# LinXueyuanStdio/LaTeX_OCR

Measured on NVIDIA H100. Metric: formula-images/sec (train step, 128x512 px, seq<=150), higher is better.
Workload: dtype bf16

## Files before the change

### include/latex_ocr_b200.h

```cpp
#ifndef LATEX_OCR_B200_H
#define LATEX_OCR_B200_H

#include <stdint.h>

#ifdef __cplusplus
extern "C" {
#endif

#define LO_F32 0
#define LO_BF16 1

#define LO_OK 0
#define LO_EINVAL (-1)
#define LO_ECUDA (-2)
#define LO_ENOTSUP (-3)

#define LO_IMPL_SIMT 0
#define LO_IMPL_TC 1

int lo_version(void);
const char* lo_last_error(void);
int64_t lo_launch_count(void);
int lo_set_option(const char* name, int value);
int lo_get_option(const char* name);
// ... 38 lines not shown
               int N, int H, int W, int Cin, int Cout, int pad, int relu, int impl, void* stream);
int lo_conv3x3_wgrad(const void* x, const void* dy, float* dw, float* db, int dt,
                     int N, int H, int W, int Cin, int Cout, int pad, int impl, void* stream);
int lo_conv_weight_flip(const void* w, void* wt, int dt, int Cin, int Cout, void* stream);
int lo_maxpool_forward(const void* x, void* y, int dt, int N, int H, int W, int C, int kh, int kw, void* stream);
int lo_maxpool_backward(const void* x, const void* y, const void* dy, void* dx, int dt,
                        int N, int H, int W, int C, int kh, int kw, void* stream);
int lo_add_table(const void* y, const float* table, void* out, int dt, int N, int64_t HWC, void* stream);
int lo_relu_mask_cast(const float* g, const void* y, void* out, int dt, int64_t n, void* stream);

int64_t lo_attention_workspace_bytes(int B, int C);
int64_t lo_decoder_workspace_bytes(int B, int C);
int lo_attention_forward(const void* att1, const void* enc, int dt, const float* att2, int64_t att2_stride,
                         const float* wf, float* alpha, int64_t alpha_stride, float* ctx,
                         float* gate_pre, int64_t gate_stride, float* gctx,
                         int B, int R, int A, int C, void* work, void* stream);
int lo_attention_forward_mask(const void* att1, const void* enc, int dt, const float* att2, int64_t att2_stride,
                              const float* wf, float* alpha, int64_t alpha_stride, float* ctx,
                              float* gate_pre, int64_t gate_stride, float* gctx, uint8_t* relu_mask_out,
                              int B, int R, int A, int C, void* work, void* stream);

int lo_attention_backward(const void* att1, const void* enc, int dt, const float* att2, const float* gate, int64_t o1_stride,
                          const float* wf, const float* alpha, int64_t alpha_stride, const float* ctx, const float* dgctx,
                          int64_t dg_stride, const float* dreg, int64_t dreg_stride, const float* sreg, int64_t sreg_stride,
                          float* de, float* datt2, float* dgp, int64_t dcat_stride, float* dctx_out, float* dwf_part,
                          const uint8_t* relu_mask, int B, int R, int A, int C, void* work, void* stream);

int64_t lo_attention_step_workspace_bytes(int B, int R, int A, int C, int dt);
int lo_attention_step_backward(const void* enc, const void* att1, int dt, const float* h, const float* att2, const void* w_enc,
                               const void* w_dec, const float* wf, const float* alpha, const float* ctx, const float* dctx,
                               const float* dalpha, float* denc, float* dh, float* g_w_enc, float* g_b_enc, float* g_w_dec,
                               float* g_b_dec, float* g_w_full, float* g_b_full, float* de, float* datt2, void* datt1,
                               int B, int R, int A, int C, int D, int impl, void* work, void* stream);

typedef struct lo_decoder_args {
  int32_t B, T, R, C, A, D, E, V;
  int32_t dt;
  int32_t impl;
  int32_t has_dropout;
  int32_t ldl;
  float alpha_c;
  int32_t rows_per_img;
  int32_t phase;
  const int32_t* bt_host;
  const int64_t* caps;
  int64_t caps_stride;
  int64_t* fed;
  const float* ss_prob;
  const float* ss_u;
  const float* ss_temp;
  const float* ss_gu;
  const void* enc;
  const void* w_enc_att; const float* b_enc_att;
  const void* wcat1; const float* bcat1;
  const float* w_full;
  const void* emb;
  const void* w_ih; const float* b_ih;
  const void* w_init; const float* b_init;
  const void* w_fc; const float* b_fc;
  void* wbwd1;
  void* wbwd2;
  void* att1;
  float* ptab;
  float* mean;
  float* hall;
  float* call;
// ... 175 lines not shown
```

### latex_ocr_b200/csrc/lo_decoder.cu

```cuda
#include "lo_common.cuh"
#include "lo_ptx.cuh"

namespace lo {

#define LO_ATT_THREADS 256
#define LO_ATT_WARPS 8
#define LO_ATT_MAXSPLIT 16

static inline int att_splits(int B) {
  int s = (444 + B - 1) / B;
  if (s < 1) s = 1;
  if (s > LO_ATT_MAXSPLIT) s = LO_ATT_MAXSPLIT;
  return s;
}

__device__ __forceinline__ float ldcg_f(const float* p) { return __ldcg(p); }

template <typename T, int NV>
__global__ void __launch_bounds__(LO_ATT_THREADS) attention_fwd_kernel(
    const T* __restrict__ att1, const T* __restrict__ enc, const float* __restrict__ att2, int64_t att2_stride,
    const float* __restrict__ wf, float* __restrict__ alpha, int64_t alpha_stride, float* __restrict__ ctx,
    float* __restrict__ gate_pre, int64_t gate_stride, float* __restrict__ gctx, bf16* __restrict__ gctx_bf, int R, int nsplit,
    int* __restrict__ counters, float* __restrict__ partials, int rpi) {
  constexpr int CH = NV * 256;
// ... 207 lines not shown
  __shared__ float s_acc[LO_ATT_WARPS][CH];
  __shared__ int s_last;
#pragma unroll
  for (int j = 0; j < NV; j++)
#pragma unroll
    for (int i = 0; i < 8; i++) s_acc[wid][(j * 32 + lane) * 8 + i] = macc[j * 8 + i];
  __syncthreads();
  float* part = partials + ((int64_t)b * nsplit + sp) * (CH + 2);
  for (int c = threadIdx.x; c < CH; c += LO_ATT_THREADS) {
    float t = 0.f;
#pragma unroll
    for (int w = 0; w < LO_ATT_WARPS; w++) t += s_acc[w][c];
    part[2 + c] = t;
  }
  __threadfence();
  __syncthreads();
  if (threadIdx.x == 0) {
    const int ticket = atomicAdd(counters + b, 1);
    s_last = (ticket == nsplit - 1);
    if (s_last) counters[b] = 0;
  }
  __syncthreads();
  if (!s_last) return;
  __threadfence();
  const float* pb = partials + (int64_t)b * nsplit * (CH + 2);
  for (int c = threadIdx.x; c < CH; c += LO_ATT_THREADS) {
    float t = 0.f;
    for (int sidx = 0; sidx < nsplit; sidx++) t += ldcg_f(pb + (int64_t)sidx * (CH + 2) + 2 + c);
    datt2[(int64_t)b * dcat_stride + c] = t * wf[c];
    if (datt2_bf) datt2_bf[(int64_t)b * dcat_stride + c] = __float2bfloat16_rn(t * wf[c]);
  }
}

template <typename T, int WACC, int ACT = 0>
__global__ void __launch_bounds__(128) datt1_kernel(const T* __restrict__ att1, const float* __restrict__ out1,
                                                     int64_t o1_row, int64_t o1_step, const float* __restrict__ de,
                                                     const float* __restrict__ wf, T* __restrict__ datt1,
                                                     float* __restrict__ dwf, int Tn, int R, int A, int nchunk, int dwf_rows) {
  constexpr int TT = 32;
  __shared__ __align__(16) float s_a2[TT][64];
  __shared__ __align__(16) float s_de[TT][32];
  __shared__ float s_w[8][64];
  const int b = blockIdx.z, a0 = blockIdx.x * 64;
  const int tx = threadIdx.x % 16, ty = threadIdx.x / 16;
  float wacc[4] = {0.f, 0.f, 0.f, 0.f};
  for (int ch = 0; ch < nchunk; ch++) {
  const int r0 = (blockIdx.y * nchunk + ch) * 32;
  if (r0 >= R) break;
  float x[4][4], nx[4][4], acc[4][4];
#pragma unroll
  for (int i = 0; i < 4; i++) {
    const int r = r0 + ty * 4 + i;
#pragma unroll
    for (int j = 0; j < 4; j++) {
      acc[i][j] = 0.f;
      x[i][j] = (r < R) ? ldf(att1 + ((int64_t)b * R + r) * A + a0 + tx * 4 + j) : -INFINITY;
      nx[i][j] = -x[i][j];
    }
  }
  for (int t0 = 0; t0 < Tn; t0 += TT) {
    for (int i = threadIdx.x; i < TT * 64; i += 128) {
      const int tt = i / 64, a = i % 64;
      s_a2[tt][a] = (t0 + tt < Tn) ? out1[(int64_t)(t0 + tt) * o1_step + (int64_t)b * o1_row + a0 + a] : 0.f;
    }
    for (int i = threadIdx.x; i < TT * 32; i += 128) {
      const int tt = i / 32, r = i % 32;
      s_de[tt][r] = (t0 + tt < Tn && r0 + r < R) ? de[((int64_t)b * Tn + t0 + tt) * R + r0 + r] : 0.f;
    }
    __syncthreads();
#pragma unroll 4
    for (int tt = 0; tt < TT; tt++) {
      const float4 q = *reinterpret_cast<const float4*>(&s_a2[tt][tx * 4]);
      const float4 d4 = *reinterpret_cast<const float4*>(&s_de[tt][ty * 4]);
      const float a2v[4] = {q.x, q.y, q.z, q.w}, dv[4] = {d4.x, d4.y, d4.z, d4.w};
      if constexpr (ACT == 0 && WACC == 1) {
        float sc[4] = {0.f, 0.f, 0.f, 0.f};
#pragma unroll
        for (int i = 0; i < 4; i++)
#pragma unroll
          for (int j = 0; j < 4; j++) {
            const bool on = a2v[j] > nx[i][j];
            if (on) { acc[i][j] += dv[i]; sc[j] += dv[i]; }
          }
#pragma unroll
        for (int j = 0; j < 4; j++) wacc[j] = fmaf(a2v[j], sc[j], wacc[j]);
      } else
#pragma unroll
      for (int i = 0; i < 4; i++)
#pragma unroll
        for (int j = 0; j < 4; j++) {
          if constexpr (ACT == 0) {
            const bool on = a2v[j] > nx[i][j];
            acc[i][j] += on ? dv[i] : 0.f;
          } else {
            const float pre = x[i][j] + a2v[j];
            const float post = tanhf(pre);
            acc[i][j] = fmaf(dv[i], 1.f - post * post, acc[i][j]);
            if (WACC) wacc[j] = fmaf(dv[i], post, wacc[j]);
          }
        }
    }
    __syncthreads();
  }
  float wv[4];
#pragma unroll
  for (int j = 0; j < 4; j++) wv[j] = wf[a0 + tx * 4 + j];
#pragma unroll
  for (int i = 0; i < 4; i++) {
    const int r = r0 + ty * 4 + i;
    if (r >= R) continue;
#pragma unroll
    for (int j = 0; j < 4; j++) stf(datt1 + ((int64_t)b * R + r) * A + a0 + tx * 4 + j, acc[i][j] * wv[j]);
  }
  if constexpr (WACC != 0 && ACT == 0) {
#pragma unroll
    for (int i = 0; i < 4; i++)
      if (r0 + ty * 4 + i < R) {
#pragma unroll
        for (int j = 0; j < 4; j++) wacc[j] = fmaf(x[i][j], acc[i][j], wacc[j]);
      }
  }
  }
  if (!WACC) return;
#pragma unroll
  for (int j = 0; j < 4; j++) s_w[ty][tx * 4 + j] = wacc[j];
  __syncthreads();
  if (threadIdx.x < 64) {
    float t = 0.f;
#pragma unroll
    for (int k = 0; k < 8; k++) t += s_w[k][threadIdx.x];
    s_w[0][threadIdx.x] = t;
  }
  if (!dwf_rows) {
    if (threadIdx.x < 64) atomicAdd(dwf + a0 + threadIdx.x, s_w[0][threadIdx.x]);
    return;
  }
  cl_sync();
  if (cl_rank() == 0 && threadIdx.x < 64) dwf[(int64_t)b * A + a0 + threadIdx.x] += cl_sum(&s_w[0][threadIdx.x]);
  cl_sync();
}

template <typename T>
__global__ void mean_rows_kernel(const T* __restrict__ enc, float* __restrict__ mean, int R, int C, int rpi) {
  const int b = blockIdx.y, c = blockIdx.x * blockDim.x + threadIdx.x;
  if (c >= C) return;
  float s = 0.f;
  for (int r = 0; r < R; r++) s += ldf(enc + ((int64_t)(b / rpi) * R + r) * C + c);
  mean[(int64_t)b * C + c] = s / (float)R;
}
template <typename T>
__global__ void mean_segments_kernel(const T* __restrict__ enc, float* __restrict__ mean, const int32_t* __restrict__ reg_off, int C,
                                     int rpi) {
  const int b = blockIdx.y, c = blockIdx.x * blockDim.x + threadIdx.x;
  if (c >= C) return;
  const int g0 = reg_off[b / rpi], R = reg_off[b / rpi + 1] - g0;
  float s = 0.f;
  for (int r = 0; r < R; r++) s += ldf(enc + ((int64_t)g0 + r) * C + c);
  mean[(int64_t)b * C + c] = s / (float)R;
}

struct SsStep {
  const float* prev_logits;
  int64_t lstride;
  const float* prob;
  const float* u;
  const unsigned long long* coin_state;
  int64_t ustride;
  int64_t* fed;
  bf16* hd_bf;
};

struct GumbelStep {
// ... 1071 lines not shown
  LO_CHECK_ARG(att1 && enc && att2 && wf && alpha && ctx && work, "null pointer");
  LO_CHECK_ARG(A == C && (C == 256 || C == 512 || C == 1024), "attention_dim == encoder_dim in {256,512,1024}");
  LO_CHECK_ARG(B > 0 && B <= 512 && R > 0, "B in 1..512, R > 0");
  LO_CHECK_ARG(att2_stride % 4 == 0, "att2 rows must be 16-byte aligned");
  LO_CHECK_ARG(!relu_mask_out || g_opt_att_pipe, "mask bits are written by the TMA-ring kernel (option att_pipe=1)");
  return attention_forward_launch(att1, enc, dt, att2, att2_stride, wf, alpha, alpha_stride, ctx, gate_pre, gate_stride, gctx, nullptr,
                                  B, R, C, work, (cudaStream_t)stream, 1, relu_mask_out, 1);
}

int lo_attention_backward(const void* att1, const void* enc, int dt, const float* att2, const float* gate, int64_t o1_stride,
                          const float* wf, const float* alpha, int64_t alpha_stride, const float* ctx, const float* dgctx,
                          int64_t dg_stride, const float* dreg, int64_t dreg_stride, const float* sreg, int64_t sreg_stride, float* de,
                          float* datt2, float* dgp, int64_t dcat_stride, float* dctx_out, float* dwf_part, const uint8_t* relu_mask,
                          int B, int R, int A, int C, void* work, void* stream) {
  LO_CHECK_ARG(att1 && enc && att2 && wf && alpha && ctx && dgctx && de && datt2 && work, "null pointer");
  LO_CHECK_ARG(A == C && (C == 256 || C == 512 || C == 1024), "attention_dim == encoder_dim in {256,512,1024}");
  LO_CHECK_ARG(B > 0 && B <= 512 && R > 0, "B in 1..512, R > 0");
  LO_CHECK_ARG(g_opt_att_pipe, "stand-alone attention backward runs on the TMA-ring kernel (option att_pipe=1)");
  AttBwdArgs x{att1, enc, att2, gate, o1_stride, wf, alpha, alpha_stride, ctx, dgctx, dg_stride, dreg, dreg_stride, sreg, sreg_stride,
               de, datt2, dgp, dcat_stride, nullptr, nullptr, dctx_out, B, R, work, dwf_part, 0, 0, relu_mask};
  x.abi = 1;
  return attention_bwd_pipe(x, dt, C, (cudaStream_t)stream);
}

static inline int64_t step_ws_align(int64_t n) { return (n + 255) & ~(int64_t)255; }

int64_t lo_attention_step_workspace_bytes(int B, int R, int A, int C, int dt) {
  if (B < 1 || R < 1 || A < 1 || C < 1) return 0;
  const int64_t es = dt == LO_F32 ? 4 : 2;
  return step_ws_align(lo_attention_workspace_bytes(B, C)) + 2 * step_ws_align((int64_t)B * A * 4) + step_ws_align((int64_t)B * R * 4) +
         step_ws_align((int64_t)B * 4) + step_ws_align((int64_t)B * R * A * es) + step_ws_align((int64_t)A * C * 2);
}

int lo_attention_step_backward(const void* enc, const void* att1, int dt, const float* h, const float* att2, const void* w_enc,
                               const void* w_dec, const float* wf, const float* alpha, const float* ctx, const float* dctx,
                               const float* dalpha, float* denc, float* dh, float* g_w_enc, float* g_b_enc, float* g_w_dec, float* g_b_dec,
                               float* g_w_full, float* g_b_full, float* de, float* datt2, void* datt1, int B, int R, int A, int C, int D,
                               int impl, void* work, void* stream) {
  LO_CHECK_ARG(enc && att1 && h && att2 && w_enc && w_dec && wf && alpha && ctx && dctx && work, "null pointer");
  LO_CHECK_ARG(dt == LO_F32 || dt == LO_BF16, "dt must be LO_F32 or LO_BF16");
  LO_CHECK_ARG(impl == LO_IMPL_SIMT || impl == LO_IMPL_TC, "impl must be LO_IMPL_SIMT or LO_IMPL_TC");
  LO_CHECK_ARG(A == C && (C == 256 || C == 512 || C == 1024), "attention_dim == encoder_dim in {256,512,1024}");
  LO_CHECK_ARG(B > 0 && B <= 512 && R > 0 && D > 0, "B in 1..512, R > 0, D > 0");
  LO_CHECK_ARG((((uintptr_t)enc | (uintptr_t)att1 | (uintptr_t)datt1) & 15) == 0,
               "enc, att1 and datt1 must be 16-byte aligned (bulk copies, 16-byte stores)");
  LO_CHECK_ARG(g_opt_att_pipe, "stand-alone attention backward runs on the TMA-ring kernel (option att_pipe=1)");
  cudaStream_t st = (cudaStream_t)stream;
  const int64_t es = dt == LO_F32 ? 4 : 2;
  const int64_t BR = (int64_t)B * R;
  char* w = (char*)work + step_ws_align(lo_attention_workspace_bytes(B, C));
  float* ws_dwf = (float*)w;     w += step_ws_align((int64_t)B * A * 4);
  float* ws_de = (float*)w;      w += step_ws_align(BR * 4);
  float* ws_datt2 = (float*)w;   w += step_ws_align((int64_t)B * A * 4);
  float* ws_sreg = (float*)w;    w += step_ws_align((int64_t)B * 4);
  void* ws_datt1 = w;            w += step_ws_align(BR * A * es);
  bf16* ws_wet = (bf16*)w;
  float* de_ = de ? de : ws_de;
  float* datt2_ = datt2 ? datt2 : ws_datt2;
  const bool need_d1 = denc || g_w_enc || g_b_enc || datt1;
  void* d1 = datt1 ? datt1 : ws_datt1;
  const bool tc = impl == LO_IMPL_TC && dt == LO_BF16 && tc_available();
  if (dalpha) {
    sreg_kernel<<<cdiv(B, 8), 256, 0, st>>>(alpha, dalpha, R, 0, ws_sreg, B, 1, R);
    LO_LAUNCH_OK();
  }
  if (g_w_full) LO_CUDA(cudaMemsetAsync(ws_dwf, 0, (size_t)B * A * 4, st));
// ... 180 lines not shown
    LO_TRY(tc_gemm_tn(dcat_bf + d.A + d.C, d.O1, gctx_bf, d.C, a->g_w_ih + d.E, d.E + d.C, d.G, d.C, d.T * d.B, st));
  } else {
    LO_TRY(gemm_tn(a->dcat + d.A + d.C, LO_F32, d.O1, a->gctx, LO_F32, d.C, a->g_w_ih + d.E, LO_F32, d.E + d.C, d.G, d.C, d.T * d.B, 0,
                   LO_IMPL_SIMT, st));
  }
  LO_TRY(colsum(a->dcat + d.A + d.C, LO_F32, a->g_b_ih, d.T * d.B, d.G, d.O1, 0, st));
  const int64_t* in_tok = a->ss_prob ? a->fed : a->caps;
  const int64_t in_stride = a->ss_prob ? (int64_t)d.T : a->caps_stride;
  if (tc) {
    const int Vp = (d.V + 7) / 8 * 8;
    onehot_kernel<<<LO_NUM_SMS * 8, 256, 0, st>>>(in_tok, in_stride, work_dlen(a), bv.onehot, d.B, d.T, Vp);
    LO_LAUNCH_OK();
    LO_CUDA(cudaMemsetAsync(a->dptab, 0, (size_t)d.V * d.G * 4, st));
    LO_TRY(tc_gemm_tn(bv.onehot, Vp, dcat_bf + d.A + d.C, d.O1, a->dptab, d.G, d.V, d.G, d.T * d.B, st));
  } else {
    dim3 grid(cdiv(d.G, 256), d.V);
    dptab_kernel<<<grid, 256, 0, st>>>(a->dcat, d.O1, (int64_t)d.B * d.O1, d.A + d.C, in_tok, in_stride, work_dlen(a), a->dptab,
                                       d.B, d.T, d.G);
    LO_LAUNCH_OK();
  }
  if (tc && d.E % 64 == 0 && d.G % 64 == 0 && d.V >= 64) {
    LO_TRY(lo_cast(a->dptab, LO_F32, bv.dptab, LO_BF16, (int64_t)d.V * d.G, stream));
    transpose_kernel<bf16><<<dim3(cdiv(d.E, 32), cdiv(d.G, 32)), dim3(32, 8), 0, st>>>((const bf16*)a->w_ih, d.E + d.C, bv.wihT, d.G, d.G, d.E);
    LO_LAUNCH_OK();
    LO_TRY(tc_gemm_nt(bv.dptab, d.G, bv.wihT, d.G, a->g_emb, LO_F32, d.E, d.V, d.E, d.G, nullptr, 0, 0, st));
    LO_CUDA(cudaMemset2DAsync(a->g_w_ih, (size_t)(d.E + d.C) * 4, 0, (size_t)d.E * 4, d.G, st));
    LO_TRY(tc_gemm_tn(bv.dptab, d.G, (const bf16*)a->emb, d.E, a->g_w_ih, d.E + d.C, d.G, d.E, d.V, st));
  } else {
    LO_TRY(gemm_nn(a->dptab, LO_F32, d.G, a->w_ih, dt, d.E + d.C, a->g_emb, LO_F32, d.E, d.V, d.E, d.G, 0, LO_IMPL_SIMT, st));
    LO_TRY(gemm_tn(a->dptab, LO_F32, d.G, a->emb, dt, d.E, a->g_w_ih, LO_F32, d.E + d.C, d.G, d.E, d.V, 0, LO_IMPL_SIMT, st));
  }
  LO_CUDA(cudaMemsetAsync(a->g_b_full, 0, 4, st));
  const bool pipe_dwf = g_opt_att_pipe && !att_mask_at(a, 0);
  if (!g_opt_det) {
    dim3 grid(d.A / 64, cdiv(d.R, 32), d.B);
    if (g_opt_att_pipe) {
      LO_TRY(colsum(a->dmean, LO_F32, a->g_w_full, d.B, d.A, d.A, 0, st));
    } else {
      LO_CUDA(cudaMemsetAsync(a->g_w_full, 0, (size_t)d.A * 4, st));
    }
    if (pipe_dwf) {
      LO_DISPATCH_DT(dt, T, (datt1_kernel<T, 0><<<grid, 128, 0, st>>>((const T*)a->att1, a->out1, d.O1, (int64_t)d.B * d.O1, a->de,
                                                                       a->w_full, (T*)a->datt1, nullptr, d.T, d.R, d.A, 1, 0)));
    } else if (g_opt_att_pipe) {
      LO_DISPATCH_DT(dt, T, (datt1_kernel<T, 2><<<grid, 128, 0, st>>>((const T*)a->att1, a->out1, d.O1, (int64_t)d.B * d.O1, a->de,
                                                                       a->w_full, (T*)a->datt1, a->g_w_full, d.T, d.R, d.A, 1, 0)));
    } else {
      LO_DISPATCH_DT(dt, T, (datt1_kernel<T, 1><<<grid, 128, 0, st>>>((const T*)a->att1, a->out1, d.O1, (int64_t)d.B * d.O1, a->de,
                                                                       a->w_full, (T*)a->datt1, a->g_w_full, d.T, d.R, d.A, 1, 0)));
    }
    LO_LAUNCH_OK();
  } else {
    const int nch = cdiv(cdiv(d.R, 32), 16);
    static bool attr = false;
    if (!attr) {
      LO_CUDA(cudaFuncSetAttribute(datt1_kernel<float, 1>, cudaFuncAttributeNonPortableClusterSizeAllowed, 1));
      LO_CUDA(cudaFuncSetAttribute(datt1_kernel<bf16, 1>, cudaFuncAttributeNonPortableClusterSizeAllowed, 1));
      LO_CUDA(cudaFuncSetAttribute(datt1_kernel<float, 2>, cudaFuncAttributeNonPortableClusterSizeAllowed, 1));
      LO_CUDA(cudaFuncSetAttribute(datt1_kernel<bf16, 2>, cudaFuncAttributeNonPortableClusterSizeAllowed, 1));
      attr = true;
    }
    dim3 grid(d.A / 64, cdiv(d.R, 32 * nch), d.B);
    const dim3 cl(1, grid.y, 1);
    if (pipe_dwf) {
      LO_DISPATCH_DT(dt, T, (datt1_kernel<T, 0><<<grid, 128, 0, st>>>((const T*)a->att1, a->out1, d.O1, (int64_t)d.B * d.O1, a->de,
                                                                       a->w_full, (T*)a->datt1, nullptr, d.T, d.R, d.A, nch, 0)));
    } else if (g_opt_att_pipe) {
      LO_DISPATCH_DT(dt, T, LO_CUDA(launch_cluster(datt1_kernel<T, 2>, grid, dim3(128), 0, st, cl, false, (const T*)a->att1,
                                                   (const float*)a->out1, (int64_t)d.O1, (int64_t)d.B * d.O1, (const float*)a->de,
                                                   (const float*)a->w_full, (T*)a->datt1, a->dmean, d.T, d.R, d.A, nch, 1)));
    } else {
      LO_CUDA(cudaMemsetAsync(a->dmean, 0, (size_t)d.B * d.A * 4, st));
      LO_DISPATCH_DT(dt, T, LO_CUDA(launch_cluster(datt1_kernel<T, 1>, grid, dim3(128), 0, st, cl, false, (const T*)a->att1,
                                                   (const float*)a->out1, (int64_t)d.O1, (int64_t)d.B * d.O1, (const float*)a->de,
                                                   (const float*)a->w_full, (T*)a->datt1, a->dmean, d.T, d.R, d.A, nch, 1)));
    }
    LO_LAUNCH_OK();
    LO_TRY(colsum(a->dmean, LO_F32, a->g_w_full, d.B, d.A, d.A, 0, st));
  }
  if (tc) {
    LO_CUDA(cudaMemsetAsync(a->g_w_enc_att, 0, (size_t)d.A * d.C * 4, st));
    LO_TRY(tc_gemm_tn((const bf16*)a->datt1, d.A, (const bf16*)a->enc, d.C, a->g_w_enc_att, d.C, d.A, d.C, d.B * d.R, st));
    transpose_kernel<bf16><<<dim3(cdiv(d.C, 32), cdiv(d.A, 32)), dim3(32, 8), 0, st>>>((const bf16*)a->w_enc_att, d.C, wet_bf, d.A, d.A, d.C);
    LO_LAUNCH_OK();
    LO_TRY(tc_gemm_nt((const bf16*)a->datt1, d.A, wet_bf, d.A, a->denc, LO_F32, d.C, d.B * d.R, d.C, d.A, nullptr, 0, 0, st));
  } else {
    LO_TRY(gemm_tn(a->datt1, dt, d.A, a->enc, dt, d.C, a->g_w_enc_att, LO_F32, d.C, d.A, d.C, d.B * d.R, 0, LO_IMPL_SIMT, st));
    LO_TRY(gemm_nn(a->datt1, dt, d.A, a->w_enc_att, dt, d.C, a->denc, LO_F32, d.C, d.B * d.R, d.C, d.A, 0, LO_IMPL_SIMT, st));
  }
  LO_TRY(colsum(a->datt1, dt, a->g_b_enc_att, d.B * d.R, d.A, d.A, 0, st));
  if (tc && d.C % 8 == 0) {
    const int Rp = (int)rpad8(d.R);
    cast_pad_rows_kernel<<<LO_NUM_SMS * 8, 256, 0, st>>>(a->alphas, bv.alphas, BT, d.R, Rp);
    LO_LAUNCH_OK();
    cast_tb_to_bt_kernel<<<LO_NUM_SMS * 8, 256, 0, st>>>(a->dctx, bv.dctx, d.T, d.B, d.C);
    LO_LAUNCH_OK();
    LO_TRY(tc_gemm_tn_batched(bv.alphas, Rp, (int64_t)d.T * Rp, bv.dctx, d.C, (int64_t)d.T * d.C, a->denc, d.C, (int64_t)d.R * d.C, d.R,
                              d.C, d.T, d.B, st));
  } else {
    GemmDesc g{d.R, d.C, d.T, 1, d.R, (int64_t)d.B * d.C, 1, d.C, d.B, (int64_t)d.T * d.R, d.C, (int64_t)d.R * d.C, nullptr, 1, 0};
    LO_TRY(gemm(a->alphas, LO_F32, a->dctx, LO_F32, a->denc, LO_F32, g, LO_IMPL_SIMT, st));
  }
  LO_TRY(gemm_tn(a->dinit, LO_F32, 2 * d.D, a->mean, LO_F32, d.C, a->g_w_init, LO_F32, d.C, 2 * d.D, d.C, d.B, 0, LO_IMPL_SIMT, st));
  LO_TRY(colsum(a->dinit, LO_F32, a->g_b_init, d.B, 2 * d.D, 2 * d.D, 0, st));
  LO_TRY(gemm_nn(a->dinit, LO_F32, 2 * d.D, a->w_init, dt, d.C, a->dmean, LO_F32, d.C, d.B, d.C, 2 * d.D, 0, LO_IMPL_SIMT, st));
  {
    const int64_t total = (int64_t)d.B * d.R * d.C;
    add_rowbcast_kernel<<<LO_NUM_SMS * 8, 256, 0, st>>>(a->denc, a->dmean, d.R, d.C, 1.0f / (float)d.R, total);
    LO_LAUNCH_OK();
  }
// ... 78 lines not shown
```

### latex_ocr_b200/csrc/lo_tfdecoder.cuh

```cuda

namespace lo {

template <int MODE>
__device__ __forceinline__ void tf_lstm_pw_fwd_body(const float* __restrict__ z, const float* __restrict__ ptab,
                                                    const int64_t* __restrict__ tok, int64_t tok_stride, int V,
                                                    const float* __restrict__ c_prev, float* __restrict__ gates, float* __restrict__ c_out,
                                                    float* __restrict__ h_out, bf16* __restrict__ h_bf, int64_t xh_stride,
                                                    const float* __restrict__ keep, float* __restrict__ hd_out, bf16* __restrict__ hd_bf,
                                                    int nrows, int D, int t_idx, const SsStep& ss, const GumbelStep& gs) {
  pdl_wait();
  pdl_trigger();
  const int idx = blockIdx.x * blockDim.x + threadIdx.x;
  int64_t tk_ss = 0;
  if constexpr (MODE != 0) {
    const bool live = idx < nrows * D;
    ss_block_tokens<MODE>(tok, tok_stride, nrows, D, V, 0, t_idx, ss, gs, live, live ? idx / D : 0, tk_ss);
  }
  if (idx >= nrows * D) return;
  const int b = idx / D, j = idx % D;
  int64_t tk = V;
  if constexpr (MODE != 0) {
    tk = tk_ss;
    if (tk < 0) tk = 0;
    if (tk >= V) tk = V - 1;
// ... 604 lines not shown
    LO_CUDA(launch_pdl(tf_lstm_pw_bwd_kernel, dim3(cdiv((long)d.B * d.D, 256)), dim3(256), (size_t)0, st, w.dxh, (int64_t)d.XH, d.O,
                       (const float*)w.dhc, (int64_t)(d.D + d.C), a->keep_h ? a->keep_h + rowt * d.D : (const float*)nullptr, w.dc,
                       (const float*)(w.gates + rowt * d.G), (const float*)(w.call + rowt * d.D), (const float*)(w.call + rown * d.D),
                       w.dz + rowt * d.G, w.dz_bf ? w.dz_bf + rowt * d.G : (bf16*)nullptr, d.B, d.D));
    LO_LAUNCH_OK();
    LO_TRY(tf_nt(a, w.dz + rowt * d.G, w.dz_bf ? w.dz_bf + rowt * d.G : nullptr, d.G, w.wb6, d.G, w.dxh, d.XH, d.B, d.XH, d.G, nullptr, 1, st));
  }
  const float* H32 = a->keep_h ? w.hd : w.xh + (int64_t)d.B * d.XH + d.O;
  const bf16* Hbf = a->keep_h ? w.hd_bf : (w.xh_bf ? w.xh_bf + (int64_t)d.B * d.XH + d.O : nullptr);
  const int64_t ldH = a->keep_h ? d.D : d.XH;
  const float* O32 = w.xh + (int64_t)d.B * d.XH;
  const bf16* Obf = w.xh_bf ? w.xh_bf + (int64_t)d.B * d.XH : nullptr;
  LO_TRY(tf_tn(a, w.dz, w.dz_bf, d.G, w.xh, w.xh_bf, d.XH, a->g_w_lstm + d.E, d.LW, d.G, d.XH, TB, st));
  {
    const int64_t* tok = a->ss_prob ? a->fed : a->formula;
    const int64_t tok_stride = a->ss_prob ? (int64_t)d.T : a->formula_stride;
    if (g_opt_det) {
      tf_dptab_kernel<<<dim3(cdiv(d.G, TF_DPT_COLS), d.V + 1), 256, 0, st>>>(w.dz, tok, tok_stride, w.dptab, d.B, d.T, d.G, d.V);
    } else {
      LO_CUDA(cudaMemsetAsync(w.dptab, 0, (size_t)(d.V + 1) * d.G * 4, st));
      tf_dptab_scatter_kernel<<<LO_NUM_SMS * 8, 256, 0, st>>>(w.dz, tok, tok_stride, w.dptab, d.B, d.T, d.G, d.V);
    }
  }
  LO_LAUNCH_OK();
  LO_TRY(gemm_nn(w.dptab, LO_F32, d.G, a->w_lstm, dt, d.LW, a->g_emb, LO_F32, d.E, d.V + 1, d.E, d.G, 0, LO_IMPL_SIMT, st));
  LO_TRY(gemm_tn(w.dptab, LO_F32, d.G, a->emb, dt, d.E, a->g_w_lstm, LO_F32, d.LW, d.G, d.E, d.V + 1, 0, LO_IMPL_SIMT, st));
  LO_TRY(colsum(w.dptab, LO_F32, a->g_b_lstm, d.V + 1, d.G, d.G, 0, st));
  LO_TRY(tf_tn(a, w.dout2, w.dout2_bf, d.DW, H32, Hbf, ldH, a->g_w_cat2, d.D, d.A, d.D, TB, st));
  LO_TRY(tf_tn(a, w.dout2 + d.A, w.dout2_bf ? w.dout2_bf + d.A : nullptr, d.DW, H32, Hbf, ldH, a->g_w_cat2 + (int64_t)d.A * d.D, d.D, d.O,
               d.D, TB, st));
  LO_TRY(tf_tn(a, w.dout2 + d.A, w.dout2_bf ? w.dout2_bf + d.A : nullptr, d.DW, w.ctx, w.ctx_bf, d.C, a->g_w_oc, d.C, d.O, d.C, TB, st));
  LO_TRY(tf_tn(a, w.dlogits, w.dlogits_bf, d.Vl, O32, Obf, d.XH, a->g_w_y, d.O, d.V, d.O, TB, st));
  LO_TRY(colsum(w.dbeta_acc, LO_F32, a->g_beta, d.B, d.A, d.A, 0, st));
  {
    dim3 grid(d.A / 64, cdiv(d.R, 32), d.B);
    LO_DISPATCH_DT(dt, T, (datt1_kernel<T, 0, 1><<<grid, 128, 0, st>>>((const T*)w.att_img, w.out2, d.N2, (int64_t)d.B * d.N2, w.de, a->beta,
                                                                            (T*)w.datt_img, nullptr, d.T, d.R, d.A, 1, 0)));
    LO_LAUNCH_OK();
  }
  const int BR = d.B * d.R;
  if (dt == LO_BF16) {
    LO_TRY(tf_tn(a, nullptr, (const bf16*)w.datt_img, d.A, nullptr, (const bf16*)a->enc, d.C, a->g_w_img, d.C, d.A, d.C, BR, st));
    LO_TRY(gemm_nt(w.datt_img, LO_BF16, d.A, w.wimgT, LO_BF16, d.A, a->denc, LO_F32, d.C, BR, d.C, d.A, nullptr, 0, 0, a->impl, st));
  } else {
    LO_TRY(gemm_tn(w.datt_img, LO_F32, d.A, a->enc, LO_F32, d.C, a->g_w_img, LO_F32, d.C, d.A, d.C, BR, 0, LO_IMPL_SIMT, st));
    LO_TRY(gemm_nn(w.datt_img, LO_F32, d.A, a->w_img, LO_F32, d.C, a->denc, LO_F32, d.C, BR, d.C, d.A, 0, LO_IMPL_SIMT, st));
  }
  {
    GemmDesc g{d.R, d.C, d.T, 1, d.R, (int64_t)d.B * d.C, 1, d.C, d.B, (int64_t)d.T * d.R, d.C, (int64_t)d.R * d.C, nullptr, 1, 0};
    LO_TRY(gemm(a->alphas, LO_F32, w.dctx, LO_F32, a->denc, LO_F32, g, LO_IMPL_SIMT, st));
  }
  const int IW = 2 * d.D + d.O;
  tf_init_bwd_kernel<<<cdiv((long)d.B * IW, 256), 256, 0, st>>>(w.dc, w.dxh, d.XH, w.sinit, w.dinit, d.B, d.D, d.O);
  LO_LAUNCH_OK();
  LO_TRY(gemm_tn(w.dinit, LO_F32, IW, w.mean, LO_F32, d.C, a->g_w_init, LO_F32, d.C, IW, d.C, d.B, 0, LO_IMPL_SIMT, st));
  LO_TRY(colsum(w.dinit, LO_F32, a->g_b_init, d.B, IW, IW, 0, st));
  LO_TRY(gemm_nn(w.dinit, LO_F32, IW, a->w_init, dt, d.C, w.dmean, LO_F32, d.C, d.B, d.C, IW, 0, LO_IMPL_SIMT, st));
  {
    const int64_t total = (int64_t)d.B * d.R * d.C;
    add_rowbcast_kernel<<<LO_NUM_SMS * 8, 256, 0, st>>>(a->denc, w.dmean, d.R, d.C, 1.0f / (float)d.R, total);
    LO_LAUNCH_OK();
  }
  return LO_OK;
}

int lo_tfdec_greedy(const lo_tfdec_args* a, int64_t end_id, int max_steps, int64_t* tokens, int32_t* fin_hist, void* stream) {
  LO_TRY(tf_check(a, true));
  TfDecode f(a);
  return greedy_loop(f, end_id, max_steps, tokens, fin_hist, (cudaStream_t)stream);
}

int lo_tfdec_beam(const lo_tfdec_args* a, int64_t end_id, int max_steps, int64_t* ids, int64_t* parents, int32_t* fin_hist, float* logp,
// ... 14 lines not shown
```

Before: 2541.

## Double-buffer datt1 kernel with cp.async and widen per-thread tile

Rewrites the datt1 backward sweep kernel to use 64 threads, each owning a 4x8 tile instead of 4x4. The T-chunk loads of a2 and de now go through double-buffered cp.async, so the next stage's global loads overlap compute on the current one. Row chunks are flattened into a single pipelined loop, and att1 and datt1 move with vector loads and stores. Launches are consolidated into a datt1_sweep helper and exposed through a new public API. The trade-off is more registers per thread and fewer threads per block, which relies on more blocks per SM to keep occupancy up.

```diff
diff --git a/include/latex_ocr_b200.h b/include/latex_ocr_b200.h
--- a/include/latex_ocr_b200.h
+++ b/include/latex_ocr_b200.h
@@ -94,6 +94,9 @@
                                const float* dalpha, float* denc, float* dh, float* g_w_enc, float* g_b_enc, float* g_w_dec,
                                float* g_b_dec, float* g_w_full, float* g_b_full, float* de, float* datt2, void* datt1,
                                int B, int R, int A, int C, int D, int impl, void* work, void* stream);
+
+int lo_datt1_sweep(const void* att1, int dt, const float* a2, int64_t a2_row, int64_t a2_step, const float* de, const float* wf,
+                   void* datt1, float* dwf, int B, int T, int R, int A, int wacc, int act, void* stream);
 
 typedef struct lo_decoder_args {
   int32_t B, T, R, C, A, D, E, V;
diff --git a/latex_ocr_b200/csrc/lo_decoder.cu b/latex_ocr_b200/csrc/lo_decoder.cu
--- a/latex_ocr_b200/csrc/lo_decoder.cu
+++ b/latex_ocr_b200/csrc/lo_decoder.cu
@@ -263,112 +263,210 @@
   }
 }
 
+constexpr int DATT1_THREADS = 64, DATT1_TT = 32;
+
+__device__ __forceinline__ void cp_async4(float* dst, const float* src, bool ok) {
+  asm volatile("cp.async.ca.shared.global [%0], [%1], 4, %2;" ::"r"(smem_u32(dst)), "l"(src), "r"(ok ? 4 : 0) : "memory");
+}
+__device__ __forceinline__ void cp_async16(float* dst, const float* src, bool ok) {
+  asm volatile("cp.async.cg.shared.global [%0], [%1], 16, %2;" ::"r"(smem_u32(dst)), "l"(src), "r"(ok ? 16 : 0) : "memory");
+}
+__device__ __forceinline__ void ld4f(const float* p, float v[4]) {
+  const float4 q = *reinterpret_cast<const float4*>(p);
+  v[0] = q.x; v[1] = q.y; v[2] = q.z; v[3] = q.w;
+}
+__device__ __forceinline__ void ld4f(const bf16* p, float v[4]) {
+  const uint2 q = *reinterpret_cast<const uint2*>(p);
+  const float2 lo = __bfloat1622float2(*reinterpret_cast<const __nv_bfloat162*>(&q.x));
+  const float2 hi = __bfloat1622float2(*reinterpret_cast<const __nv_bfloat162*>(&q.y));
+  v[0] = lo.x; v[1] = lo.y; v[2] = hi.x; v[3] = hi.y;
+}
+__device__ __forceinline__ void st4f(float* p, const float v[4]) { *reinterpret_cast<float4*>(p) = make_float4(v[0], v[1], v[2], v[3]); }
+__device__ __forceinline__ void st4f(bf16* p, const float v[4]) {
+  const __nv_bfloat162 lo = __floats2bfloat162_rn(v[0], v[1]), hi = __floats2bfloat162_rn(v[2], v[3]);
+  *reinterpret_cast<uint2*>(p) = make_uint2(*reinterpret_cast<const uint32_t*>(&lo), *reinterpret_cast<const uint32_t*>(&hi));
+}
+
 template <typename T, int WACC, int ACT = 0>
-__global__ void __launch_bounds__(128) datt1_kernel(const T* __restrict__ att1, const float* __restrict__ out1,
-                                                     int64_t o1_row, int64_t o1_step, const float* __restrict__ de,
-                                                     const float* __restrict__ wf, T* __restrict__ datt1,
-                                                     float* __restrict__ dwf, int Tn, int R, int A, int nchunk, int dwf_rows) {
-  constexpr int TT = 32;
-  __shared__ __align__(16) float s_a2[TT][64];
-  __shared__ __align__(16) float s_de[TT][32];
+__global__ void __launch_bounds__(DATT1_THREADS, 8) datt1_kernel(const T* __restrict__ att1, const float* __restrict__ out1,
+                                                                 int64_t o1_row, int64_t o1_step, const float* __restrict__ de,
+                                                                 const float* __restrict__ wf, T* __restrict__ datt1,
+                                                                 float* __restrict__ dwf, int Tn, int R, int A, int nchunk,
+                                                                 int dwf_rows) {
+  constexpr int TT = DATT1_TT;
+  __shared__ __align__(16) float s_a2[2][TT][64];
+  __shared__ __align__(16) float s_de[2][TT][32];
   __shared__ float s_w[8][64];
-  const int b = blockIdx.z, a0 = blockIdx.x * 64;
-  const int tx = threadIdx.x % 16, ty = threadIdx.x / 16;
-  float wacc[4] = {0.f, 0.f, 0.f, 0.f};
-  for (int ch = 0; ch < nchunk; ch++) {
-  const int r0 = (blockIdx.y * nchunk + ch) * 32;
-  if (r0 >= R) break;
-  float x[4][4], nx[4][4], acc[4][4];
-#pragma unroll
-  for (int i = 0; i < 4; i++) {
-    const int r = r0 + ty * 4 + i;
-#pragma unroll
-    for (int j = 0; j < 4; j++) {
-      acc[i][j] = 0.f;
-      x[i][j] = (r < R) ? ldf(att1 + ((int64_t)b * R + r) * A + a0 + tx * 4 + j) : -INFINITY;
-      nx[i][j] = -x[i][j];
-    }
-  }
-  for (int t0 = 0; t0 < Tn; t0 += TT) {
-    for (int i = threadIdx.x; i < TT * 64; i += 128) {
-      const int tt = i / 64, a = i % 64;
-      s_a2[tt][a] = (t0 + tt < Tn) ? out1[(int64_t)(t0 + tt) * o1_step + (int64_t)b * o1_row + a0 + a] : 0.f;
-    }
-    for (int i = threadIdx.x; i < TT * 32; i += 128) {
-      const int tt = i / 32, r = i % 32;
-      s_de[tt][r] = (t0 + tt < Tn && r0 + r < R) ? de[((int64_t)b * Tn + t0 + tt) * R + r0 + r] : 0.f;
-    }
+  const int b = blockIdx.z, a0 = blockIdx.x * 64, tid = threadIdx.x;
+  const int tx = tid % 8, ty = tid / 8;
+  const int rb = blockIdx.y * nchunk * 32;
+  const int nch = min(nchunk, (R - rb + 31) / 32), nt = (Tn + TT - 1) / TT, nq = nch * nt;
+  const float* a2b = out1 + (int64_t)b * o1_row + a0;
+  const float* deb = de + (int64_t)b * Tn * R;
+  const bool vec = ((((uintptr_t)out1 | (uintptr_t)de) & 15) | ((o1_row | o1_step) & 3) | (R & 3)) == 0;
+  auto stage = [&](int q) {
+    const int t0 = (q % nt) * TT, r0 = rb + (q / nt) * 32, s = q & 1;
+    if (vec) {
+#pragma unroll
+      for (int k = 0; k < 8; k++) {
+        const int tt = tid / 16 + 4 * k, c = (tid % 16) * 4;
+        const bool ok = t0 + tt < Tn;
+        cp_async16(&s_a2[s][tt][c], ok ? a2b + (int64_t)(t0 + tt) * o1_step + c : out1, ok);
+      }
+#pragma unroll
+      for (int k = 0; k < 4; k++) {
+        const int tt = tid / 8 + 8 * k, r = (tid % 8) * 4;
+        const bool ok = t0 + tt < Tn && r0 + r < R;
+        cp_async16(&s_de[s][tt][r], ok ? deb + (int64_t)(t0 + tt) * R + r0 + r : de, ok);
+      }
+    } else {
+      for (int tt = 0; tt < TT; tt++) {
+        const bool ok = t0 + tt < Tn;
+        cp_async4(&s_a2[s][tt][tid], ok ? a2b + (int64_t)(t0 + tt) * o1_step + tid : out1, ok);
+      }
+      for (int k = 0; k < TT / 2; k++) {
+        const int tt = tid / 32 + 2 * k, r = tid % 32;
+        const bool ok = t0 + tt < Tn && r0 + r < R;
+        cp_async4(&s_de[s][tt][r], ok ? deb + (int64_t)(t0 + tt) * R + r0 + r : de, ok);
+      }
+    }
+    asm volatile("cp.async.commit_group;" ::: "memory");
+  };
+  float wacc[8];
+#pragma unroll
+  for (int j = 0; j < 8; j++) wacc[j] = 0.f;
+  float nx[4][8], acc[4][8];
+  if (nq > 0) stage(0);
+  for (int q = 0; q < nq; q++) {
+    const int tc = q % nt, r0 = rb + (q / nt) * 32, s = q & 1;
+    if (tc == 0) {
+#pragma unroll
+      for (int i = 0; i < 4; i++) {
+        const int r = r0 + ty * 4 + i;
+        float v[8];
+        if (r < R) {
+          ld4f(att1 + ((int64_t)b * R + r) * A + a0 + tx * 4, v);
+          ld4f(att1 + ((int64_t)b * R + r) * A + a0 + 32 + tx * 4, v + 4);
+        } else {
+#pragma unroll
+          for (int j = 0; j < 8; j++) v[j] = -INFINITY;
+        }
+#pragma unroll
+        for (int j = 0; j < 8; j++) {
+          acc[i][j] = 0.f;
+          nx[i][j] = -v[j];
+        }
+      }
+    }
+    if (q + 1 < nq) stage(q + 1);
+    else asm volatile("cp.async.commit_group;" ::: "memory");
+    asm volatile("cp.async.wait_group 1;" ::: "memory");
     __syncthreads();
-#pragma unroll 4
-    for (int tt = 0; tt < TT; tt++) {
-      const float4 q = *reinterpret_cast<const float4*>(&s_a2[tt][tx * 4]);
-      const float4 d4 = *reinterpret_cast<const float4*>(&s_de[tt][ty * 4]);
-      const float a2v[4] = {q.x, q.y, q.z, q.w}, dv[4] = {d4.x, d4.y, d4.z, d4.w};
+    const int nstep = min(TT, Tn - tc * TT);
+#pragma unroll 1
+    for (int tt = 0; tt < nstep; tt++) {
+      float a2v[8], dv[4];
+      ld4f(&s_a2[s][tt][tx * 4], a2v);
+      ld4f(&s_a2[s][tt][32 + tx * 4], a2v + 4);
+      ld4f(&s_de[s][tt][ty * 4], dv);
       if constexpr (ACT == 0 && WACC == 1) {
-        float sc[4] = {0.f, 0.f, 0.f, 0.f};
+        float sc[8];
+#pragma unroll
+        for (int j = 0; j < 8; j++) sc[j] = 0.f;
 #pragma unroll
         for (int i = 0; i < 4; i++)
 #pragma unroll
-          for (int j = 0; j < 4; j++) {
-            const bool on = a2v[j] > nx[i][j];
-            if (on) { acc[i][j] += dv[i]; sc[j] += dv[i]; }
+          for (int j = 0; j < 8; j++)
+            if (a2v[j] > nx[i][j]) { acc[i][j] += dv[i]; sc[j] += dv[i]; }
+#pragma unroll
+        for (int j = 0; j < 8; j++) wacc[j] = fmaf(a2v[j], sc[j], wacc[j]);
+      } else {
+#pragma unroll
+        for (int i = 0; i < 4; i++)
+#pragma unroll
+          for (int j = 0; j < 8; j++) {
+            if constexpr (ACT == 0) {
+              if (a2v[j] > nx[i][j]) acc[i][j] += dv[i];
+            } else {
+              const float post = tanhf(a2v[j] - nx[i][j]);
+              acc[i][j] = fmaf(dv[i], 1.f - post * post, acc[i][j]);
+            }
           }
-#pragma unroll
-        for (int j = 0; j < 4; j++) wacc[j] = fmaf(a2v[j], sc[j], wacc[j]);
-      } else
-#pragma unroll
-      for (int i = 0; i < 4; i++)
-#pragma unroll
-        for (int j = 0; j < 4; j++) {
-          if constexpr (ACT == 0) {
-            const bool on = a2v[j] > nx[i][j];
-            acc[i][j] += on ? dv[i] : 0.f;
-          } else {
-            const float pre = x[i][j] + a2v[j];
-            const float post = tanhf(pre);
-            acc[i][j] = fmaf(dv[i], 1.f - post * post, acc[i][j]);
-            if (WACC) wacc[j] = fmaf(dv[i], post, wacc[j]);
-          }
+      }
+    }
+    __syncthreads();
+    if (tc == nt - 1) {
+      float wv[8];
+#pragma unroll
+      for (int j = 0; j < 4; j++) {
+        wv[j] = wf[a0 + tx * 4 + j];
+        wv[4 + j] = wf[a0 + 32 + tx * 4 + j];
+      }
+#pragma unroll
+      for (int i = 0; i < 4; i++) {
+        const int r = r0 + ty * 4 + i;
+        if (r >= R) continue;
+        float o[8];
+#pragma unroll
+        for (int j = 0; j < 8; j++) o[j] = acc[i][j] * wv[j];
+        st4f(datt1 + ((int64_t)b * R + r) * A + a0 + tx * 4, o);
+        st4f(datt1 + ((int64_t)b * R + r) * A + a0 + 32 + tx * 4, o + 4);
+        if constexpr (WACC != 0 && ACT == 0) {
+#pragma unroll
+          for (int j = 0; j < 8; j++) wacc[j] = fmaf(-nx[i][j], acc[i][j], wacc[j]);
         }
-    }
-    __syncthreads();
-  }
-  float wv[4];
-#pragma unroll
-  for (int j = 0; j < 4; j++) wv[j] = wf[a0 + tx * 4 + j];
-#pragma unroll
-  for (int i = 0; i < 4; i++) {
-    const int r = r0 + ty * 4 + i;
-    if (r >= R) continue;
-#pragma unroll
-    for (int j = 0; j < 4; j++) stf(datt1 + ((int64_t)b * R + r) * A + a0 + tx * 4 + j, acc[i][j] * wv[j]);
-  }
-  if constexpr (WACC != 0 && ACT == 0) {
-#pragma unroll
-    for (int i = 0; i < 4; i++)
-      if (r0 + ty * 4 + i < R) {
-#pragma unroll
-        for (int j = 0; j < 4; j++) wacc[j] = fmaf(x[i][j], acc[i][j], wacc[j]);
       }
-  }
+    }
   }
   if (!WACC) return;
 #pragma unroll
-  for (int j = 0; j < 4; j++) s_w[ty][tx * 4 + j] = wacc[j];
+  for (int j = 0; j < 4; j++) {
+    s_w[ty][tx * 4 + j] = wacc[j];
+    s_w[ty][32 + tx * 4 + j] = wacc[4 + j];
+  }
   __syncthreads();
-  if (threadIdx.x < 64) {
-    float t = 0.f;
-#pragma unroll
-    for (int k = 0; k < 8; k++) t += s_w[k][threadIdx.x];
-    s_w[0][threadIdx.x] = t;
-  }
+  float t = 0.f;
+#pragma unroll
+  for (int k = 0; k < 8; k++) t += s_w[k][tid];
+  s_w[0][tid] = t;
   if (!dwf_rows) {
-    if (threadIdx.x < 64) atomicAdd(dwf + a0 + threadIdx.x, s_w[0][threadIdx.x]);
+    atomicAdd(dwf + a0 + tid, t);
     return;
   }
   cl_sync();
-  if (cl_rank() == 0 && threadIdx.x < 64) dwf[(int64_t)b * A + a0 + threadIdx.x] += cl_sum(&s_w[0][threadIdx.x]);
+  if (cl_rank() == 0) dwf[(int64_t)b * A + a0 + tid] += cl_sum(&s_w[0][tid]);
   cl_sync();
+}
+
+template <typename T, int WACC, int ACT>
+static int datt1_launch(const T* att1, const float* a2, int64_t a2_row, int64_t a2_step, const float* de, const float* wf,
+                        T* datt1, float* dwf, int B, int Tn, int R, int A, cudaStream_t st) {
+  if (WACC && g_opt_det) {
+    static bool attr = false;
+    if (!attr) {
+      LO_CUDA(cudaFuncSetAttribute(datt1_kernel<T, WACC, ACT>, cudaFuncAttributeNonPortableClusterSizeAllowed, 1));
+      attr = true;
+    }
+    const int nch = cdiv(cdiv(R, 32), 16);
+    const dim3 grid(A / 64, cdiv(R, 32 * nch), B);
+    LO_CUDA(launch_cluster(datt1_kernel<T, WACC, ACT>, grid, dim3(DATT1_THREADS), 0, st, dim3(1, grid.y, 1), false, att1, a2, a2_row,
+                           a2_step, de, wf, datt1, dwf, Tn, R, A, nch, 1));
+  } else {
+    datt1_kernel<T, WACC, ACT><<<dim3(A / 64, cdiv(R, 32), B), DATT1_THREADS, 0, st>>>(att1, a2, a2_row, a2_step, de, wf, datt1, dwf, Tn, R,
+                                                                             A, 1, 0);
+  }
+  LO_LAUNCH_OK();
+  return LO_OK;
+}
+
+static int datt1_sweep(const void* att1, int dt, const float* a2, int64_t a2_row, int64_t a2_step, const float* de, const float* wf,
+                       void* datt1, float* dwf, int B, int Tn, int R, int A, int wacc, int act, cudaStream_t st) {
+  LO_DISPATCH_DT(dt, T,
+                 const T* x = (const T*)att1; T* y = (T*)datt1;
+                 if (act) return datt1_launch<T, 0, 1>(x, a2, a2_row, a2_step, de, wf, y, nullptr, B, Tn, R, A, st);
+                 if (wacc == 1) return datt1_launch<T, 1, 0>(x, a2, a2_row, a2_step, de, wf, y, dwf, B, Tn, R, A, st);
+                 if (wacc == 2) return datt1_launch<T, 2, 0>(x, a2, a2_row, a2_step, de, wf, y, dwf, B, Tn, R, A, st);
+                 return datt1_launch<T, 0, 0>(x, a2, a2_row, a2_step, de, wf, y, nullptr, B, Tn, R, A, st));
 }
 
 template <typename T>
@@ -1506,6 +1604,16 @@
          step_ws_align((int64_t)B * 4) + step_ws_align((int64_t)B * R * A * es) + step_ws_align((int64_t)A * C * 2);
 }
 
+int lo_datt1_sweep(const void* att1, int dt, const float* a2, int64_t a2_row, int64_t a2_step, const float* de, const float* wf,
+                   void* datt1, float* dwf, int B, int T, int R, int A, int wacc, int act, void* stream) {
+  LO_CHECK_ARG(att1 && a2 && de && wf && datt1, "null pointer");
+  LO_CHECK_ARG(B > 0 && T > 0 && R > 0 && A > 0 && A % 64 == 0, "B, T, R > 0 and A a positive multiple of 64");
+  LO_CHECK_ARG(wacc >= 0 && wacc <= 2 && (act == 0 || act == 1) && !(act && wacc), "wacc in 0..2, act in 0..1, act = 1 only with wacc = 0");
+  LO_CHECK_ARG(!wacc || dwf, "wacc > 0 needs dwf");
+  LO_CHECK_ARG((((uintptr_t)att1 | (uintptr_t)datt1) & 15) == 0, "att1 and datt1 must be 16-byte aligned (vector loads and stores)");
+  return datt1_sweep(att1, dt, a2, a2_row, a2_step, de, wf, datt1, dwf, B, T, R, A, wacc, act, (cudaStream_t)stream);
+}
+
 int lo_attention_step_backward(const void* enc, const void* att1, int dt, const float* h, const float* att2, const void* w_enc,
                                const void* w_dec, const float* wf, const float* alpha, const float* ctx, const float* dctx,
                                const float* dalpha, float* denc, float* dh, float* g_w_enc, float* g_b_enc, float* g_w_dec, float* g_b_dec,
@@ -1752,50 +1860,19 @@
   }
   LO_CUDA(cudaMemsetAsync(a->g_b_full, 0, 4, st));
   const bool pipe_dwf = g_opt_att_pipe && !att_mask_at(a, 0);
+  const int wacc = pipe_dwf ? 0 : g_opt_att_pipe ? 2 : 1;
   if (!g_opt_det) {
-    dim3 grid(d.A / 64, cdiv(d.R, 32), d.B);
     if (g_opt_att_pipe) {
       LO_TRY(colsum(a->dmean, LO_F32, a->g_w_full, d.B, d.A, d.A, 0, st));
     } else {
       LO_CUDA(cudaMemsetAsync(a->g_w_full, 0, (size_t)d.A * 4, st));
     }
-    if (pipe_dwf) {
-      LO_DISPATCH_DT(dt, T, (datt1_kernel<T, 0><<<grid, 128, 0, st>>>((const T*)a->att1, a->out1, d.O1, (int64_t)d.B * d.O1, a->de,
-                                                                       a->w_full, (T*)a->datt1, nullptr, d.T, d.R, d.A, 1, 0)));
-    } else if (g_opt_att_pipe) {
-      LO_DISPATCH_DT(dt, T, (datt1_kernel<T, 2><<<grid, 128, 0, st>>>((const T*)a->att1, a->out1, d.O1, (int64_t)d.B * d.O1, a->de,
-                                                                       a->w_full, (T*)a->datt1, a->g_w_full, d.T, d.R, d.A, 1, 0)));
-    } else {
-      LO_DISPATCH_DT(dt, T, (datt1_kernel<T, 1><<<grid, 128, 0, st>>>((const T*)a->att1, a->out1, d.O1, (int64_t)d.B * d.O1, a->de,
-                                                                       a->w_full, (T*)a->datt1, a->g_w_full, d.T, d.R, d.A, 1, 0)));
-    }
-    LO_LAUNCH_OK();
+    LO_TRY(datt1_sweep(a->att1, dt, a->out1, d.O1, (int64_t)d.B * d.O1, a->de, a->w_full, a->datt1, a->g_w_full, d.B, d.T, d.R,
+                       d.A, wacc, 0, st));
   } else {
-    const int nch = cdiv(cdiv(d.R, 32), 16);
-    static bool attr = false;
-    if (!attr) {
-      LO_CUDA(cudaFuncSetAttribute(datt1_kernel<float, 1>, cudaFuncAttributeNonPortableClusterSizeAllowed, 1));
-      LO_CUDA(cudaFuncSetAttribute(datt1_kernel<bf16, 1>, cudaFuncAttributeNonPortableClusterSizeAllowed, 1));
-      LO_CUDA(cudaFuncSetAttribute(datt1_kernel<float, 2>, cudaFuncAttributeNonPortableClusterSizeAllowed, 1));
-      LO_CUDA(cudaFuncSetAttribute(datt1_kernel<bf16, 2>, cudaFuncAttributeNonPortableClusterSizeAllowed, 1));
-      attr = true;
-    }
-    dim3 grid(d.A / 64, cdiv(d.R, 32 * nch), d.B);
-    const dim3 cl(1, grid.y, 1);
-    if (pipe_dwf) {
-      LO_DISPATCH_DT(dt, T, (datt1_kernel<T, 0><<<grid, 128, 0, st>>>((const T*)a->att1, a->out1, d.O1, (int64_t)d.B * d.O1, a->de,
-                                                                       a->w_full, (T*)a->datt1, nullptr, d.T, d.R, d.A, nch, 0)));
-    } else if (g_opt_att_pipe) {
-      LO_DISPATCH_DT(dt, T, LO_CUDA(launch_cluster(datt1_kernel<T, 2>, grid, dim3(128), 0, st, cl, false, (const T*)a->att1,
-                                                   (const float*)a->out1, (int64_t)d.O1, (int64_t)d.B * d.O1, (const float*)a->de,
-                                                   (const float*)a->w_full, (T*)a->datt1, a->dmean, d.T, d.R, d.A, nch, 1)));
-    } else {
-      LO_CUDA(cudaMemsetAsync(a->dmean, 0, (size_t)d.B * d.A * 4, st));
-      LO_DISPATCH_DT(dt, T, LO_CUDA(launch_cluster(datt1_kernel<T, 1>, grid, dim3(128), 0, st, cl, false, (const T*)a->att1,
-                                                   (const float*)a->out1, (int64_t)d.O1, (int64_t)d.B * d.O1, (const float*)a->de,
-                                                   (const float*)a->w_full, (T*)a->datt1, a->dmean, d.T, d.R, d.A, nch, 1)));
-    }
-    LO_LAUNCH_OK();
+    if (!g_opt_att_pipe) LO_CUDA(cudaMemsetAsync(a->dmean, 0, (size_t)d.B * d.A * 4, st));
+    LO_TRY(datt1_sweep(a->att1, dt, a->out1, d.O1, (int64_t)d.B * d.O1, a->de, a->w_full, a->datt1, a->dmean, d.B, d.T, d.R, d.A,
+                       wacc, 0, st));
     LO_TRY(colsum(a->dmean, LO_F32, a->g_w_full, d.B, d.A, d.A, 0, st));
   }
   if (tc) {
diff --git a/latex_ocr_b200/csrc/lo_tfdecoder.cuh b/latex_ocr_b200/csrc/lo_tfdecoder.cuh
--- a/latex_ocr_b200/csrc/lo_tfdecoder.cuh
+++ b/latex_ocr_b200/csrc/lo_tfdecoder.cuh
@@ -660,12 +660,8 @@
   LO_TRY(tf_tn(a, w.dout2 + d.A, w.dout2_bf ? w.dout2_bf + d.A : nullptr, d.DW, w.ctx, w.ctx_bf, d.C, a->g_w_oc, d.C, d.O, d.C, TB, st));
   LO_TRY(tf_tn(a, w.dlogits, w.dlogits_bf, d.Vl, O32, Obf, d.XH, a->g_w_y, d.O, d.V, d.O, TB, st));
   LO_TRY(colsum(w.dbeta_acc, LO_F32, a->g_beta, d.B, d.A, d.A, 0, st));
-  {
-    dim3 grid(d.A / 64, cdiv(d.R, 32), d.B);
-    LO_DISPATCH_DT(dt, T, (datt1_kernel<T, 0, 1><<<grid, 128, 0, st>>>((const T*)w.att_img, w.out2, d.N2, (int64_t)d.B * d.N2, w.de, a->beta,
-                                                                            (T*)w.datt_img, nullptr, d.T, d.R, d.A, 1, 0)));
-    LO_LAUNCH_OK();
-  }
+  LO_TRY(datt1_sweep(w.att_img, dt, w.out2, d.N2, (int64_t)d.B * d.N2, w.de, a->beta, w.datt_img, nullptr, d.B, d.T, d.R, d.A, 0, 1,
+                     st));
   const int BR = d.B * d.R;
   if (dt == LO_BF16) {
     LO_TRY(tf_tn(a, nullptr, (const bf16*)w.datt_img, d.A, nullptr, (const bf16*)a->enc, d.C, a->g_w_img, d.C, d.A, d.C, BR, st));
```

Result: no change. 2593 (median of 6 runs) (+2.0%).
